# ctu-mrs/mrs_multirotor_simulator

Hardware: NVIDIA B200
Metric: UAV-steps/s (RK4+control+collisions) at 1M UAVs (higher is better)
Workload: dtype f64

## Files before the change

mrs_multirotor_simulator_b200/csrc/api.cu:

```cuda
#include <dlfcn.h>
#include <nccl.h>

#include <algorithm>
#include <cmath>
#include <cstdarg>
#include <cstdio>
#include <cstring>
#include <functional>
#include <map>
#include <memory>
#include <string>
#include <type_traits>
#include <utility>
#include <vector>

#include "internal.h"
#include "params.h"

static thread_local char g_err[512] = "";

static int fail(int code, const char* fmt, ...) {
  va_list ap;
  va_start(ap, fmt);
  vsnprintf(g_err, sizeof(g_err), fmt, ap);
  va_end(ap);
  return code;
}

#define CU(call)                                                                                              \
  do {                                                                                                        \
    cudaError_t e_ = (call);                                                                                  \
    if (e_ != cudaSuccess) return fail(MRSB_ERR_CUDA, "%s failed: %s (%s:%d)", #call, cudaGetErrorString(e_), __FILE__, __LINE__); \
  } while (0)

struct NcclApi {
  void* lib = nullptr;
  ncclResult_t (*GetUniqueId)(ncclUniqueId*)                                                         = nullptr;
  ncclResult_t (*CommInitRank)(ncclComm_t*, int, ncclUniqueId, int)                                  = nullptr;
  ncclResult_t (*CommDestroy)(ncclComm_t)                                                            = nullptr;
  ncclResult_t (*AllGather)(const void*, void*, size_t, ncclDataType_t, ncclComm_t, cudaStream_t)    = nullptr;
  ncclResult_t (*Broadcast)(const void*, void*, size_t, ncclDataType_t, int, ncclComm_t, cudaStream_t) = nullptr;
// ... 167 lines not shown
  bool                 equal_shards = true;

  bool                 p2p       = false;
  double*              gbuf[2]   = {nullptr, nullptr};
  uint32_t*            d_gbox[2] = {nullptr, nullptr};
  int64_t              pass_no   = 0;
  bool                 wrote_since_pass = false;
  std::vector<int32_t> pending_geom[2];
  PeerView             pv[2]{};
  PeerView             pv_local{};
  P2PCtl               p2pctl{};
  unsigned long long*  d_flags   = nullptr;
  unsigned long long** d_peer_flags = nullptr;
  std::vector<void*>   ipc_opened;
  Mem<int, true>       h_status;

  cudaStream_t up_stream = nullptr, down_stream = nullptr;
  Mem<double>  d_up[2];
  Mem<double>  d_snap[2];
  cudaEvent_t  ev_up[2] = {nullptr, nullptr}, ev_applied[2] = {nullptr, nullptr}, ev_snap[2] = {nullptr, nullptr}, ev_down[2] = {nullptr, nullptr};
  uint64_t     n_up = 0, n_down = 0;
  Mem<int32_t> d_sub_idx;
  int64_t      n_sub = 0;

  Graph pass[2], tick[2];
  bool  graph_failed = false;

  bool     lists_on            = false;
  int      steps_since_pass    = 0;
  bool     positions_touched   = true;
  int      rebuild_own         = 0;
  int64_t  list_passes         = 0;
  int64_t  rebuilds_counted    = 0;
  Mem<uint32_t, true> h_one;
  Mem<unsigned long long, true> h_until;

  struct NbWorkspace {
    Mem<double>             pos, vel;
    Mem<uint32_t>           bucket, rank, count, begin;
    Mem<double4>            rec;
    Mem<unsigned long long> scan;
  } nb;

  struct Snapshot {
    Mem<unsigned char> mem;
    bool    filled       = false;
    int32_t uniform_mode = MRSB_INPUT_UNKNOWN;
    bool    any_moment   = false;
  };
  std::map<int32_t, Snapshot> snapshots;
  int32_t                     next_snapshot = 1;

  int64_t n_steps = 0, n_passes = 0, n_launches = 0;
  int     step_info[4] = {0, 0, 0, 0};
};

static std::string set_key(const ParamSet& s) {
  return std::string(reinterpret_cast<const char*>(&s), sizeof(ParamSet));
}

static int intern_set(mrsb_sim* h, const ParamSet& s) {
  const std::string key = set_key(s);
  auto              it  = h->set_index.find(key);
  if (it != h->set_index.end()) return it->second;
  const int id = int(h->sets.size());
  h->sets.push_back(s);
// ... 23 lines not shown
  s.cp.rate_kp = cp.rate_kp, s.cp.rate_kd = cp.rate_kd, s.cp.rate_ki = cp.rate_ki;
  s.cp.att_kp = cp.att_kp, s.cp.att_kd = cp.att_kd, s.cp.att_ki = cp.att_ki, s.cp.att_max_rate_roll_pitch = cp.att_max_rate_roll_pitch,
  s.cp.att_max_rate_yaw = cp.att_max_rate_yaw;
  s.cp.vel_kp = cp.vel_kp, s.cp.vel_kd = cp.vel_kd, s.cp.vel_ki = cp.vel_ki, s.cp.vel_max_acceleration = cp.vel_max_acceleration;
  s.cp.pos_kp = cp.pos_kp, s.cp.pos_kd = cp.pos_kd, s.cp.pos_ki = cp.pos_ki, s.cp.pos_max_velocity = cp.pos_max_velocity;
  return s;
}

static int collect_param_sets(mrsb_sim* h) {
  const int n_sets = int(h->sets.size());
  if (n_sets <= 32) return MRSB_OK;
  std::vector<int> refs(size_t(n_sets), 0);
  for (int32_t id : h->pset_host) refs[size_t(id)]++;
  int live = 0;
  for (int r : refs) live += r > 0;
  if (2 * live > n_sets) return MRSB_OK;
  std::vector<int>      remap(size_t(n_sets), -1);
  std::vector<ParamSet> kept;
  kept.reserve(size_t(live));
  h->set_index.clear();
  for (int k = 0; k < n_sets; k++) {
    if (!refs[size_t(k)]) continue;
    remap[size_t(k)] = int(kept.size());
    h->set_index[set_key(h->sets[size_t(k)])] = int(kept.size());
    kept.push_back(h->sets[size_t(k)]);
  }
  h->sets.swap(kept);
  for (int32_t& id : h->pset_host) id = remap[size_t(id)];
  CU(cudaMemcpyAsync(h->d_pset, h->pset_host.data(), sizeof(int32_t) * h->pset_host.size(), cudaMemcpyHostToDevice, h->stream));
  CU(cudaStreamSynchronize(h->stream));
  return MRSB_OK;
}

static int flush_params(mrsb_sim* h) {
  if (!h->params_dirty) return MRSB_OK;
  int rc = collect_param_sets(h);
  if (rc) return rc;
  const int    n_sets = int(h->sets.size());
  const size_t cap    = size_t(std::max(16, 2 * n_sets));
  rc                  = h->d_params.grow(size_t(n_sets), cap, h->stream);
  if (rc) return rc;
  h->ds.params = h->d_params.get();
  rc           = h->d_takeoff0.grow(size_t(n_sets), cap, h->stream);
  if (rc) return rc;
  std::vector<DevParams> host(n_sets);
  std::vector<uint8_t>   takeoff0(size_t(n_sets), 0);
  for (int k = 0; k < n_sets; k++) {
    mrsb_derive(h->sets[k].mp, h->sets[k].cp, &host[k]);
    takeoff0[size_t(k)] = h->sets[k].mp.takeoff_patch_enabled != 0;
  }
  CU(cudaMemcpyAsync(h->d_params.get(), host.data(), sizeof(DevParams) * n_sets, cudaMemcpyHostToDevice, h->stream));
  CU(cudaMemcpyAsync(h->d_takeoff0.get(), takeoff0.data(), size_t(n_sets), cudaMemcpyHostToDevice, h->stream));
  CU(cudaStreamSynchronize(h->stream));
  h->filt_dt = -1.0;
  for (Bucket& b : h->buckets) {
    int nm = -1, ps = -2;
    for (int64_t k = 0; k < b.count; k++) {
      const int64_t e  = h->inv_host.empty() ? b.slot0 + k : h->inv_host[size_t(b.slot0 + k)];
      const int     id = h->pset_host[size_t(h->ds.shard_begin + e)];
      const int     m  = h->sets[size_t(id)].mp.n_motors;
      if (nm == -1) nm = m;
      if (nm != m) nm = 0;
      if (ps == -2) ps = id;
      if (ps != id) ps = -1;
      if (nm == 0 && ps == -1) break;
    }
    b.nm   = nm > 0 ? nm : 0;
    b.pset = ps >= 0 ? ps : -1;
    if (b.pset >= 0) b.params = host[size_t(b.pset)];
  }
  h->params_dirty = false;
  return MRSB_OK;
}

static int ensure_filt(mrsb_sim* h, double dt) {
  if (h->filt_dt == dt) return MRSB_OK;
  h->n_launches += launch_prep_params(h->d_params.get(), int(h->sets.size()), dt, h->stream);
  for (Bucket& b : h->buckets)
    if (b.pset >= 0) CU(cudaMemcpyAsync(&b.params.filt, &h->d_params.get()[b.pset].filt, sizeof(double), cudaMemcpyDeviceToHost, h->stream));
  CU(cudaStreamSynchronize(h->stream));
  h->filt_dt = dt;
  return MRSB_OK;
}

static int ensure_stage(mrsb_sim* h, size_t bytes) {
  return h->d_stage.grow(bytes, std::max<size_t>(bytes, 1 << 16), h->stream);
}

static int stage_idx(mrsb_sim* h, int64_t n, const int32_t* idx, const int32_t** out) {
  *out = nullptr;
  if (n < 0 || n > h->ds.n && !idx) return fail(MRSB_ERR_INVALID, "n=%lld outside 0..%lld", (long long)n, (long long)h->ds.n);
  if (!idx || n == 0) return MRSB_OK;
  for (int64_t k = 0; k < n; k++)
    if (idx[k] < 0 || idx[k] >= h->ds.n) return fail(MRSB_ERR_INVALID, "idx[%lld]=%d outside 0..%lld", (long long)k, idx[k], (long long)h->ds.n - 1);
  int rc = h->d_idx.grow(size_t(n), std::max<size_t>(size_t(n), 1024), h->stream);
  if (rc) return rc;
  CU(cudaMemcpyAsync(h->d_idx.get(), idx, sizeof(int32_t) * n, cudaMemcpyHostToDevice, h->stream));
  *out = h->d_idx.get();
  return MRSB_OK;
}

struct HostRows {
  const double* rows;
  int           width;
};
// ... 132 lines not shown
      ParamSet s = h->sets[old];
      edit(s, k);
      id        = intern_set(h, canonical(s.mp, s.cp));
      memo[key] = id;
      const mrsb_model_params &a = h->sets[size_t(old)].mp, &b = h->sets[size_t(id)].mp;
      if (a.arm_length != b.arm_length || a.prop_radius != b.prop_radius || a.mass != b.mass) geometry = true;
    }
    ids[size_t(k)]                                 = id;
    h->pset_host[size_t(h->ds.shard_begin + i)] = id;
  }
  if (geometry && h->ds.n_global > h->ds.n && !h->p2p) {
    for (int64_t k = n - 1; k >= 0; k--) h->pset_host[size_t(h->ds.shard_begin + (idx ? idx[k] : k))] = olds[size_t(k)];
    return fail(MRSB_ERR_STATE, "arm length / propeller radius / mass of a sharded handle can only change while its peers read them from this "
                                "GPU (exchange mode 2, mrsb_comm_init_nccl with peer access)");
  }
  h->params_dirty = true;
  rc              = ensure_stage(h, sizeof(int32_t) * size_t(n));
  if (rc) return rc;
  CU(cudaMemcpyAsync(h->d_stage.get(), ids.data(), sizeof(int32_t) * size_t(n), cudaMemcpyHostToDevice, h->stream));
  h->n_launches += launch_set_pset(h->d_pset, n, d_idx, h->ds.shard_begin, reinterpret_cast<const int32_t*>(h->d_stage.get()), h->stream);
  CU(cudaStreamSynchronize(h->stream));
  if (geometry) {
    rc = flush_params(h);
    if (rc) return rc;
    rc = stage_idx(h, n, idx, &d_idx);
    if (rc) return rc;
    rc = geometry_changed(h, n, idx, d_idx);
    if (rc) return rc;
    CU(cudaStreamSynchronize(h->stream));
  }
  return MRSB_OK;
}

static void set_collision_geometry(mrsb_sim* h, bool lists) {
  DevGrid& g  = h->grid;
  h->lists_on = lists;
  double cell = lists ? 6.0 : 4.0;
  if (const char* e = getenv("MRSB_COLLISION_CELL")) cell = std::max(3.5, atof(e));
  g.inv_cell = 1.0 / cell;
  g.reach    = 0.5 * cell;
  const double r_list = g.reach * (1.0 - 1e-6);
  g.list_r2  = r_list * r_list;
  g.skin     = (r_list - 1.7320508075688775) * (1.0 - 1e-6);
  h->ds.disp_max       = lists ? &g.ctl->disp_max_bits : nullptr;
  h->positions_touched = true;
}

static void make_local_view(mrsb_sim* h) {
  PeerView& v = h->pv_local;
  v           = PeerView{};
  v.n_ranks   = 1;
  v.rank      = 0;
  v.begin[0]  = 0;
  v.begin[1]  = h->ds.n_global;
  v.pos[0]    = h->ds.gpos;
  v.geom[0]   = h->d_geom[0];
}

static int setup_p2p(mrsb_sim* h) {
  const int    G     = h->n_ranks;
  const size_t ng    = size_t(h->ds.n_global);
  h->gbuf[0]         = h->ds.gpos;
  int rc             = dalloc(h, &h->gbuf[1], 3 * ng);
  if (rc) return rc;
  CU(cudaMemcpy(h->gbuf[1], h->gbuf[0], sizeof(double) * 3 * ng, cudaMemcpyDeviceToDevice));
  rc = dalloc(h, &h->d_geom[1], 4 * ng);
  if (rc) return rc;
  CU(cudaMemcpy(h->d_geom[1], h->d_geom[0], sizeof(double) * 4 * ng, cudaMemcpyDeviceToDevice));
  for (int k = 0; k < 2; k++) {
    rc = dalloc(h, &h->d_gbox[k], 6 * size_t(h->ds.ld / 32 + 1));
    if (rc) return rc;
  }
  rc = dalloc(h, &h->d_flags, 3 * size_t(G));
  if (rc) return rc;
  rc = h->h_status.alloc(1);
  if (rc) return rc;
  *h->h_status.get() = 0;
  struct Handles {
// ... 49 lines not shown
      h->pv[k].box[r] = static_cast<const uint32_t*>(p);
      rc              = open(all[size_t(r)].geom[k], &p);
      if (rc) return rc;
      h->pv[k].geom[r] = static_cast<const double*>(p);
    }
    rc = open(all[size_t(r)].flags, &p);
    if (rc) return rc;
    pflags[size_t(r)] = static_cast<unsigned long long*>(p);
  }
  rc = dalloc(h, &h->d_peer_flags, size_t(G));
  if (rc) return rc;
  CU(cudaMemcpy(h->d_peer_flags, pflags.data(), sizeof(unsigned long long*) * G, cudaMemcpyHostToDevice));
  Mem<unsigned long long> d_tmp;
  rc = d_tmp.alloc(size_t(G));
  if (rc) return rc;
  NC(g_nccl.AllGather(d_tmp.get() + h->rank, d_tmp.get(), sizeof(unsigned long long), ncclChar, h->comm, h->stream));
  CU(cudaStreamSynchronize(h->stream));
  h->p2pctl.peer_flags = h->d_peer_flags;
  h->p2pctl.flags      = h->d_flags;
  h->p2pctl.n_ranks    = G;
  h->p2pctl.rank       = h->rank;
  h->p2pctl.status     = h->h_status.get();
  {
    const char* e    = getenv("MRSB_P2P_TIMEOUT_MS");
    h->p2pctl.budget = (e ? atoll(e) : 20000LL) * 2000000LL;
  }
  h->p2p     = true;
  h->pass_no = 0;
  h->ds.gpos = h->gbuf[1];
  h->ds.gbox = h->d_gbox[1];
  h->ds.geom = h->d_geom[1];
  h->n_launches += launch_publish_positions(h->ds, h->stream);
  h->wrote_since_pass = true;
  set_collision_geometry(h, h->grid.nl_count != nullptr);
  CU(cudaStreamSynchronize(h->stream));
  return MRSB_OK;
}

extern "C" {

const char* mrsb_last_error(void) {
  return g_err;
}
int mrsb_version(void) {
  return MRSB_VERSION_MAJOR * 1000 + MRSB_VERSION_MINOR;
}

int mrsb_destroy(mrsb_handle h) {
  if (!h) return MRSB_OK;
  cudaSetDevice(h->device);
  const cudaStream_t streams[3] = {h->stream, h->up_stream, h->down_stream};
  for (cudaStream_t s : streams)
    if (s) cudaStreamSynchronize(s);
  for (int k = 0; k < 2; k++) h->pass[k] = Graph(), h->tick[k] = Graph();
  for (void* p : h->ipc_opened) cudaIpcCloseMemHandle(p);
  if (h->comm && g_nccl.CommDestroy) g_nccl.CommDestroy(h->comm);
  for (int k = 0; k < 2; k++)
    for (cudaEvent_t e : {h->ev_up[k], h->ev_applied[k], h->ev_snap[k], h->ev_down[k]})
      if (e) cudaEventDestroy(e);
  delete h;
  for (cudaStream_t s : streams)
    if (s) cudaStreamDestroy(s);
  return MRSB_OK;
}

int mrsb_bucket_layout(int64_t n, int32_t n_types, const int32_t* type_of_local_uav, int32_t* slot_of_uav, int64_t* n_slots, int64_t* bucket_first_slot,
                       int64_t* bucket_count) {
// ... 165 lines not shown
    g.scan_tiles = scan_tiles_for(int64_t(g.n_buckets) + 3);
    g.halo_cap   = std::max<int64_t>(s.n_global - s.n, 1);
    rc = dalloc(h, &g.bucket, ng);
    if (!rc) rc = dalloc(h, &g.rank, ng);
    if (!rc) rc = dalloc(h, &g.count, size_t(g.n_buckets) + 4);
    if (!rc) rc = dalloc(h, &g.begin, size_t(g.n_buckets) + 4);
    if (!rc) rc = dalloc(h, &g.aabb, 6);
    if (!rc) rc = dalloc(h, &g.rec, 2 * ng);
    if (!rc) rc = h->pairs.grow(2 * size_t(g.pair_cap), 2 * size_t(g.pair_cap), h->stream);
    if (!rc) rc = dalloc(h, &g.counters, 4);
    if (!rc) rc = dalloc(h, &g.scan_state, size_t(g.scan_tiles) + size_t(scan_tiles_for(s.n)) + 2);
    if (!rc && s.n_global > s.n) rc = dalloc(h, &g.halo_rec, size_t(g.halo_cap));
    if (!rc && s.n_global > s.n) rc = dalloc(h, &g.halo_bucket, size_t(g.halo_cap));
    if (!rc && s.n_global > s.n) rc = dalloc(h, &g.halo_rank, size_t(g.halo_cap));
    if (!rc) rc = dalloc(h, &g.halo_n, 2);
    if (!rc && s.n_global > s.n) rc = dalloc(h, &g.halo_work, size_t(g.halo_cap / 32 + MRSB_MAX_RANKS + 1));
    if (!rc && getenv("MRSB_TIMELINE")) rc = dalloc(h, &g.tl, size_t(MRSB_TL_TICKS) * 8);
    if (!rc) rc = dalloc(h, &g.ctl, 1);
    if (!rc) rc = h->h_one.alloc(2);
    if (!rc) rc = h->h_until.alloc(1);
    if (rc) return rc;
    g.pairs       = h->pairs.get();
    g.halo_work_n = g.halo_n + 1;
    h->h_one.get()[0] = 1u;
    h->h_one.get()[1] = 0xFFFFFFFFu;
    if (s.n > 0 && !getenv("MRSB_NO_NEIGHBOUR_LISTS")) {
      g.nl_ld = s.ld;
      rc      = dalloc(h, &g.nl_count, size_t(g.nl_ld));
      if (!rc) rc = dalloc(h, &g.nl_items, size_t(MRSB_NL_CAP) * size_t(g.nl_ld));
      if (!rc) rc = dalloc(h, &g.nl_active, size_t(g.nl_ld));
      if (!rc) rc = dalloc(h, &g.act_items, size_t(MRSB_NL_CAP) * size_t(g.nl_ld));
      if (rc) return rc;
    }
    set_collision_geometry(h, g.nl_count != nullptr && s.n_global == s.n);
  }
  make_local_view(h);
  h->shard_begin_of = {s.shard_begin};
  h->shard_count_of = {s.n};
  CU(cudaStreamSynchronize(h->stream));
  *out = guard.release();
  return MRSB_OK;
}

int mrsb_sync(mrsb_handle h) {
  GUARD(h);
  CU(cudaStreamSynchronize(h->stream));
  if (h->up_stream) CU(cudaStreamSynchronize(h->up_stream));
  if (h->down_stream) CU(cudaStreamSynchronize(h->down_stream));
  return MRSB_OK;
}

static int ensure_pipeline(mrsb_sim* h) {
  if (h->d_snap[1].get()) return MRSB_OK;
  for (cudaStream_t* s : {&h->up_stream, &h->down_stream})
    if (!*s) CU(cudaStreamCreateWithFlags(s, cudaStreamNonBlocking));
  const size_t snap = 3 * size_t(std::max<int64_t>(h->ds.n, 1));
  for (int k = 0; k < 2; k++) {
    for (cudaEvent_t* e : {&h->ev_up[k], &h->ev_applied[k], &h->ev_snap[k], &h->ev_down[k]})
      if (!*e) CU(cudaEventCreateWithFlags(e, cudaEventDisableTiming));
    int rc = h->d_snap[k].grow(snap, snap, h->down_stream);
    if (rc) return rc;
  }
  return MRSB_OK;
}

int mrsb_set_input_async(mrsb_handle h, int32_t mode, const double* payload, int32_t stride) {
  GUARD(h);
// ... 1240 lines not shown
```

mrs_multirotor_simulator_b200/csrc/collide.cu:

```cuda
#include <algorithm>

#include "internal.h"

namespace {

#define DEV __device__ __forceinline__

#define NL_LIVE 0x80000000u
#define NL_CROWDED 0x40000000u

DEV unsigned long long now_ns() {
  unsigned long long t;
  asm volatile("mov.u64 %0, %globaltimer;" : "=l"(t));
  return t;
}
DEV void stamp(const DevGrid& g, int slot, unsigned long long value) {
  if (g.tl) g.tl[((g.ctl->n_passes - 1ull) % MRSB_TL_TICKS) * 8 + slot] = value;
}

DEV int cell_of(double v, double inv_cell) {
  return __double2int_rd(__dmul_rn(v, inv_cell));
}

DEV uint32_t row_hash(int cy, int cz) {
  uint32_t h = uint32_t(cy) * 0x9E3779B1u ^ (uint32_t(cz) * 0x85EBCA77u + 0x165667B1u);
  h ^= h >> 15;
  h *= 0x2C1B3C6Du;
  h ^= h >> 12;
  return h;
}

DEV unsigned long long enc(double v) {
  const unsigned long long b = (unsigned long long)__double_as_longlong(v);
  return (b >> 63) ? ~b : (b | 0x8000000000000000ull);
}
DEV double dec(unsigned long long e) {
  const unsigned long long b = (e >> 63) ? (e & 0x7fffffffffffffffull) : ~e;
  return __longlong_as_double((long long)b);
}
DEV float fdec(uint32_t e) {
  return __uint_as_float((e >> 31) ? (e & 0x7fffffffu) : ~e);
}
// ... 196 lines not shown
    double*       lp = s.gpos + 3 * gj;
    lp[0] = x, lp[1] = y, lp[2] = z;
    double2* lg = reinterpret_cast<double2*>(s.geom + 4 * gj);
    lg[0] = a, lg[1] = b;
  }
}

#define SCAN_PER_THREAD 16
#define SCAN_TILE (256 * SCAN_PER_THREAD)
#define SCAN_FLAG_A (1ull << 32)
#define SCAN_FLAG_P (2ull << 32)
template <bool HASWORK>
__global__ void __launch_bounds__(256) scan_kernel(const uint32_t* __restrict__ in, uint32_t* __restrict__ out, int64_t n, unsigned long long* state) {
  __shared__ uint32_t s_tile, s_warp[8], s_prefix;
  const uint32_t      full = 0xffffffffu;
  const int           lane = threadIdx.x & 31, wid = threadIdx.x >> 5;
  if (threadIdx.x == 0) s_tile = uint32_t(atomicAdd(&state[0], 1ull));
  __syncthreads();
  const int64_t tile = s_tile;
  const int64_t base = tile * SCAN_TILE + int64_t(threadIdx.x) * SCAN_PER_THREAD;
  uint32_t      v[SCAN_PER_THREAD];
  if (base + SCAN_PER_THREAD <= n) {
#pragma unroll
    for (int q = 0; q < SCAN_PER_THREAD / 4; q++) {
      const uint4 a = reinterpret_cast<const uint4*>(in + base)[q];
      v[4 * q] = a.x, v[4 * q + 1] = a.y, v[4 * q + 2] = a.z, v[4 * q + 3] = a.w;
    }
  } else {
#pragma unroll
    for (int k = 0; k < SCAN_PER_THREAD; k++) v[k] = base + k < n ? in[base + k] : 0u;
  }
  if (HASWORK) {
#pragma unroll
    for (int k = 0; k < SCAN_PER_THREAD; k++) v[k] = (v[k] & 0x7FFFFFFFu) != 0u ? 1u : 0u;
  }
  uint32_t mine = 0;
#pragma unroll
  for (int k = 0; k < SCAN_PER_THREAD; k++) mine += v[k];
  uint32_t incl = mine;
#pragma unroll
  for (int o = 1; o < 32; o <<= 1) {
    const uint32_t t = __shfl_up_sync(full, incl, o);
    if (lane >= o) incl += t;
  }
  if (lane == 31) s_warp[wid] = incl;
  __syncthreads();
  uint32_t warp_off = 0, total = 0;
#pragma unroll
  for (int w = 0; w < 8; w++) {
    if (w < wid) warp_off += s_warp[w];
    total += s_warp[w];
  }
  if (wid == 0) {
    volatile unsigned long long* st = state + 1;
    uint32_t                     prefix = 0;
    if (tile == 0) {
      if (lane == 0) st[0] = SCAN_FLAG_P | total;
    } else {
      if (lane == 0) st[tile] = SCAN_FLAG_A | total;
      int64_t look = tile - 1;
      while (true) {
        const int64_t      t = look - lane;
        unsigned long long w = t >= 0 ? st[t] : SCAN_FLAG_P;
        while (__any_sync(full, (w >> 32) == 0ull)) {
          if ((w >> 32) == 0ull) w = st[t];
        }
        const uint32_t pm    = __ballot_sync(full, (w >> 32) == 2ull);
// ... 176 lines not shown
  PairAcc acc;
  if (n_ball > 0) {
    const Geom Gi      = load_geom(s, gi);
    auto       process = [&](const double4& r) { process_pair(s, g, crash_mode, rebounce, gi, q.x, q.y, q.z, Gi, __double_as_longlong(r.w), r.x, r.y, r.z, acc); };
    if (n_ball <= 2) {
      for (int c = 0; c < n_ball; c++) {
        process(g.rec[h0]);
        h0 = h1;
      }
    } else {
      int64_t last = -1;
      for (int c = 0; c < n_ball; c++) {
        int64_t  best = INT64_MAX;
        uint32_t bt   = 0;
        for (int k = 0; k < 4; k++) {
          for (uint32_t t = st.lo[k]; t < st.hi[k]; t++) {
            const double4 r  = g.rec[t];
            const int64_t gj = __double_as_longlong(r.w);
            if (gj <= last || gj >= best || !in_ball(r, k)) continue;
            best = gj;
            bt   = t;
          }
        }
        if (best == INT64_MAX) break;
        process(g.rec[bt]);
        last = best;
      }
    }
  }
  store_result(s, li, acc);
  if (g.nl_count) g.nl_count[li] = (g.nl_count[li] & ~NL_LIVE) | (nonzero(acc) ? NL_LIVE : 0u);
}


__global__ void __launch_bounds__(128) build_lists_kernel(DevState s, DevGrid g) {
  if (blockIdx.x == 0 && threadIdx.x == 0) stamp(g, 7, now_ns());
  const uint32_t full  = 0xffffffffu;
  const int      lane  = threadIdx.x & 31;
  const int      k     = threadIdx.x & 3;
  const int64_t  n_rec = int64_t(g.begin[g.n_buckets]);
  const uint32_t quad  = 0xFu << (lane & ~3);
  const uint32_t below = quad & ((1u << lane) - 1u);
  const uint32_t mask  = g.n_buckets - 1;
  const bool     write_all = g.ctl->n_passes <= g.ctl->write_all_until;
  for (int64_t p0 = int64_t(blockIdx.x) * 32; p0 < n_rec; p0 += int64_t(gridDim.x) * 32) {
    const int64_t p   = p0 + (threadIdx.x >> 2);
    const bool    has = p < n_rec;
    double4       q   = make_double4(0.0, 0.0, 0.0, 0.0);
    if (has) q = g.rec[p];
    const int64_t gi   = __double_as_longlong(q.w);
    const int64_t li   = gi - s.shard_begin;
    const bool    mine = has && li >= 0 && li < s.n;
    const int cx0 = cell_of(q.x - g.reach, g.inv_cell), cy0 = cell_of(q.y - g.reach, g.inv_cell), cz0 = cell_of(q.z - g.reach, g.inv_cell);
    uint32_t  lo = 0, len = 0;
    if (mine) {
      const uint32_t b0 = (row_hash(cy0 + (k & 1), cz0 + (k >> 1)) + uint32_t(cx0)) & mask;
      lo                = g.begin[b0];
      len               = g.begin[b0 + 2] - lo;
    }
    const int      qb  = lane & ~3;
    const uint32_t lo0 = __shfl_sync(full, lo, qb), lo1 = __shfl_sync(full, lo, qb + 1), lo2 = __shfl_sync(full, lo, qb + 2), lo3 = __shfl_sync(full, lo, qb + 3);
    const uint32_t c1  = __shfl_sync(full, len, qb);
    const uint32_t c2  = c1 + __shfl_sync(full, len, qb + 1);
    const uint32_t c3  = c2 + __shfl_sync(full, len, qb + 2);
    const uint32_t tot = c3 + __shfl_sync(full, len, qb + 3);
    auto where = [&](uint32_t c, int& row) -> uint32_t {
      row = int(c >= c1) + int(c >= c2) + int(c >= c3);
      return row == 0 ? lo0 + c : (row == 1 ? lo1 + (c - c1) : (row == 2 ? lo2 + (c - c2) : lo3 + (c - c3)));
    };
    uint32_t cnt = 0;
    for (uint32_t c = uint32_t(k); __any_sync(full, c < tot); c += 8) {
      double4 r[2];
      int     row[2] = {0, 0};
#pragma unroll
      for (int u = 0; u < 2; u++)
        if (c + 4 * u < tot) r[u] = g.rec[where(c + 4 * u, row[u])];
#pragma unroll
      for (int u = 0; u < 2; u++) {
        bool    take = false;
        int32_t gj   = 0;
        if (c + 4 * u < tot) {
          gj = int32_t(__double_as_longlong(r[u].w));
          if (int64_t(gj) != gi && nf_dist2(q.x, q.y, q.z, r[u].x, r[u].y, r[u].z) < g.list_r2 && cell_of(r[u].y, g.inv_cell) == cy0 + (row[u] & 1) &&
              cell_of(r[u].z, g.inv_cell) == cz0 + (row[u] >> 1))
            take = true;
        }
        const uint32_t bal = __ballot_sync(full, take) & quad;
        if (take) {
          const uint32_t slot = cnt + __popc(bal & below);
          if (slot < MRSB_NL_CAP) g.nl_items[int64_t(slot) * g.nl_ld + li] = gj;
        }
        cnt += __popc(bal);
      }
    }
    __syncwarp();
    const bool lead = mine && k == 0;
    if (lead) {
      uint32_t live = g.nl_count[li] & NL_LIVE;
      if (cnt == 0u && (live || write_all)) {
        const int64_t sl            = slot_of(s, li);
        s.fext[tix(F3_ROWS, 0, sl)] = 0.0;
        s.fext[tix(F3_ROWS, 1, sl)] = 0.0;
        s.fext[tix(F3_ROWS, 2, sl)] = 0.0;
        live                        = 0u;
      }
      if (cnt > MRSB_NL_CAP) {
        g.nl_items[li] = int32_t(uint32_t(p));
        g.nl_count[li] = NL_CROWDED | live;
        atomicAdd(&g.ctl->n_crowded, 1u);
      } else {
        g.nl_count[li] = cnt | live;
      }
    }
  }
}

__global__ void __launch_bounds__(256) compact_kernel(DevGrid g, const uint32_t* __restrict__ slot, int64_t n) {
  const int64_t li = int64_t(blockIdx.x) * blockDim.x + threadIdx.x;
  if (li >= n) return;
  const uint32_t word = g.nl_count[li];
  const bool     work = (word & 0x7FFFFFFFu) != 0u;
  if (work) {
    const uint32_t k   = slot[li];
    g.nl_active[k]     = make_uint2(uint32_t(li), word);
    const uint32_t cnt = (word & NL_CROWDED) ? 1u : (word & ~(NL_LIVE | NL_CROWDED));
    for (uint32_t c = 0; c < cnt; c++) g.act_items[int64_t(c) * g.nl_ld + k] = g.nl_items[int64_t(c) * g.nl_ld + li];
  }
  if (li == n - 1) g.ctl->n_active = slot[li] + (work ? 1u : 0u);
}

DEV void check_crowded(const DevState& s, const DevGrid& g, int crash_mode, double rebounce, int64_t gi, uint32_t rec_index, PairAcc& acc) {
  const double4 qb = g.rec[rec_index];
  const Stencil st = stencil_of(g, qb.x, qb.y, qb.z);
  const double* qp = s.gpos + 3 * gi;
  const double  qx = qp[0], qy = qp[1], qz = qp[2];
  auto in_ball = [&](const double4& r, int k) {
    const int64_t gj = __double_as_longlong(r.w);
    if (gj == gi) return false;
    if (cell_of(r.y, g.inv_cell) != st.rcy[k] || cell_of(r.z, g.inv_cell) != st.rcz[k]) return false;
    double rx, ry, rz;
    load_pos(s, gj, rx, ry, rz);
    return nf_dist2(qx, qy, qz, rx, ry, rz) < 3.0;
  };
  const Geom Gi      = load_geom(s, gi);
  auto       process = [&](int64_t gj) {
    double rx, ry, rz;
    load_pos(s, gj, rx, ry, rz);
    process_pair(s, g, crash_mode, rebounce, gi, qx, qy, qz, Gi, gj, rx, ry, rz, acc);
  };
  int     n_ball = 0;
  int64_t h0 = 0, h1 = 0;
  for (int k = 0; k < 4; k++)
    for (uint32_t t = st.lo[k]; t < st.hi[k]; t++) {
      const double4 r = g.rec[t];
      if (!in_ball(r, k)) continue;
      if (n_ball == 0) h0 = __double_as_longlong(r.w);
      if (n_ball == 1) h1 = __double_as_longlong(r.w);
      n_ball++;
    }
  if (n_ball <= 2) {
    if (n_ball >= 1) process(h0);
    if (n_ball == 2) process(h1);
    return;
  }
  int64_t last = -1;
  for (int c = 0; c < n_ball; c++) {
    int64_t best = INT64_MAX;
    for (int k = 0; k < 4; k++)
      for (uint32_t t = st.lo[k]; t < st.hi[k]; t++) {
        const double4 r  = g.rec[t];
        const int64_t gj = __double_as_longlong(r.w);
        if (gj <= last || gj >= best || !in_ball(r, k)) continue;
        best = gj;
      }
    if (best == INT64_MAX) break;
    process(best);
    last = best;
  }
}

DEV void check_one(const DevState& s, const DevGrid& g, int crash_mode, double rebounce, uint32_t k, int64_t li, uint32_t word, const int32_t* first4) {
  const uint32_t cnt  = word & ~(NL_LIVE | NL_CROWDED);
  const bool     live = (word & NL_LIVE) || g.ctl->n_passes <= g.ctl->write_all_until;
  PairAcc acc;
  if (word & NL_CROWDED) {
    check_crowded(s, g, crash_mode, rebounce, li + s.shard_begin, uint32_t(first4[0]), acc);
  } else if (cnt) {
    const int64_t gi = li + s.shard_begin;
    const double* qp = s.gpos + 3 * gi;
    const double  qx = qp[0], qy = qp[1], qz = qp[2];
    uint32_t      hits = 0;
    for (uint32_t base = 0; base < cnt; base += 4) {
      int32_t gj[4];
      double  r[4][3];
#pragma unroll
      for (int u = 0; u < 4; u++) gj[u] = base + u < cnt ? (base == 0 ? first4[u] : g.act_items[int64_t(base + u) * g.nl_ld + k]) : -1;
#pragma unroll
      for (int u = 0; u < 4; u++) load_pos(s, int64_t(max(gj[u], 0)), r[u][0], r[u][1], r[u][2]);
#pragma unroll
      for (int u = 0; u < 4; u++)
        if (gj[u] >= 0 && nf_dist2(qx, qy, qz, r[u][0], r[u][1], r[u][2]) < 3.0) hits |= 1u << (base + u);
    }
    if (hits) {
      const Geom Gi      = load_geom(s, gi);
      auto       process = [&](uint32_t c) {
        const int64_t gj = g.act_items[int64_t(c) * g.nl_ld + k];
        double        rx, ry, rz;
        load_pos(s, gj, rx, ry, rz);
        process_pair(s, g, crash_mode, rebounce, gi, qx, qy, qz, Gi, gj, rx, ry, rz, acc);
      };
      if (__popc(hits) <= 2) {
        while (hits) {
          process(uint32_t(__ffs(int(hits)) - 1));
          hits &= hits - 1;
        }
      } else {
        int64_t last = -1;
        while (hits) {
          int64_t  best = INT64_MAX;
          uint32_t bc   = 0;
          for (uint32_t m = hits; m; m &= m - 1) {
            const uint32_t c  = uint32_t(__ffs(int(m)) - 1);
            const int64_t  gj = g.act_items[int64_t(c) * g.nl_ld + k];
            if (gj > last && gj < best) best = gj, bc = c;
          }
          if (best == INT64_MAX) break;
          process(bc);
          last = best;
          hits &= ~(1u << bc);
        }
      }
    }
  }
  const bool nz = nonzero(acc);
  if (live || nz) store_result(s, li, acc);
  else if (acc.crashed_me) s.flags[slot_of(s, li)] |= FLAG_CRASHED;
  if (nz != bool(word & NL_LIVE)) {
    const uint32_t nw = (word & ~NL_LIVE) | (nz ? NL_LIVE : 0u);
    g.nl_count[li]    = nw;
    g.nl_active[k].y  = nw;
  }
}

#ifndef MRSB_CHECK_THREADS
#define MRSB_CHECK_THREADS 256
#define MRSB_CHECK_MINB 4
#endif
__global__ void __launch_bounds__(MRSB_CHECK_THREADS, MRSB_CHECK_MINB) check_kernel(DevState s, DevGrid g, int crash_mode, double rebounce, int skip_if_rebuild) {
  if (skip_if_rebuild && g.ctl->rebuild) return;
  if (blockIdx.x == 0 && threadIdx.x == 0) stamp(g, 4, now_ns());
  const uint32_t n_active = g.ctl->n_active;
  for (uint32_t k = blockIdx.x * blockDim.x + threadIdx.x; k < n_active; k += gridDim.x * blockDim.x) {
    const uint2 e = g.nl_active[k];
    int32_t     first4[4];
#pragma unroll
    for (int u = 0; u < 4; u++) first4[u] = g.act_items[int64_t(u) * g.nl_ld + k];
    check_one(s, g, crash_mode, rebounce, k, int64_t(e.x), e.y, first4);
  }
}

__global__ void __launch_bounds__(32) decide_kernel(NlCtl* __restrict__ c, unsigned long long* __restrict__ pair_counter, double skin, int always,
                                                    cudaGraphConditionalHandle handle, int has_handle, P2PCtl p, unsigned long long* tl) {
  const uint32_t full = 0xffffffffu;
  const int      lane = threadIdx.x;
  unsigned long long* row = tl ? tl + (c->n_passes % MRSB_TL_TICKS) * 8 : nullptr;
  if (row && lane == 0) row[0] = now_ns();
  uint32_t                 bits  = c->disp_max_bits;
  const double             D_old = c->D_total;
  const uint32_t           force = c->force, valid = c->valid;
  const unsigned long long n_rebuilds = c->n_rebuilds, n_passes = c->n_passes;
  if (p.n_ranks > 1) {
    const unsigned long long epoch = c->epoch + 1ull;
    const int                slot  = int(epoch & 1ull);
    const bool               peer  = lane < p.n_ranks && lane != p.rank;
    volatile unsigned long long* theirs = peer ? p.peer_flags[lane] : nullptr;
    if (peer) theirs[p.n_ranks + 2 * p.rank + slot] = (unsigned long long)(always ? 0xFFFFFFFFu : bits);
    __threadfence_system();
    if (peer) theirs[p.rank] = epoch;
    if (row && lane == 0) row[1] = now_ns();
    uint32_t got = 0u;
    if (peer) {
      volatile const unsigned long long* mine = p.flags;
      const long long                    t0   = clock64();
      bool                               ok   = true;
      while (mine[lane] < epoch) {
        if (clock64() - t0 > p.budget) {
          *p.status = 1;
          ok        = false;
          break;
        }
// ... 224 lines not shown
```

mrs_multirotor_simulator_b200/csrc/internal.h:

```cpp
#pragma once
#include <cuda_runtime.h>
#include <stdint.h>

#include "../../include/mrsb.h"

#define MRSB_NM MRSB_MAX_MOTORS
#define MRSB_TILE 128

static __host__ __device__ __forceinline__ int64_t tix(int rows, int row, int64_t i) {
  return ((i >> 7) * rows + row) * MRSB_TILE + (i & (MRSB_TILE - 1));
}
#define ST_ROWS 18
#define VPREV_ROWS 3
#define F3_ROWS 3

#define FLAG_CRASHED 1u
#define FLAG_TAKEOFF 2u
#define FLAG_VPREV 4u
#define FLAG_HAD_INPUT 256u
#define FLAG_FF_VEL_HDG_RATE 16u
#define FLAG_FF_VEL_HDG 32u
#define FLAG_FF_ACC_HDG_RATE 64u
#define FLAG_FF_ACC_HDG 128u

// ... 58 lines not shown
#define STEP_OPT_IMU 1u
#define STEP_OPT_GPOS 2u
#define STEP_OPT_NEED_INPUT 4u

#define MRSB_MAX_RANKS 16
struct PeerView {
  int32_t         n_ranks, rank;
  int64_t         begin[MRSB_MAX_RANKS + 1];
  const double*   pos[MRSB_MAX_RANKS];
  const uint32_t* box[MRSB_MAX_RANKS];
  const double*   geom[MRSB_MAX_RANKS];
};

struct P2PCtl {
  unsigned long long* const* peer_flags;
  unsigned long long*        flags;
  int32_t                    n_ranks, rank;
  int*                       status;
  long long                  budget;
};

#define MRSB_NL_CAP 8
#define MRSB_TL_TICKS 4096
struct NlCtl {
  uint32_t disp_max_bits;
  uint32_t force;
  uint32_t valid;
  uint32_t n_active;
  uint32_t n_crowded;
  uint32_t rebuild;
  double   D_total;
  unsigned long long n_rebuilds, n_passes, epoch ;
  unsigned long long write_all_until;
};

struct DevGrid {
  uint32_t  n_buckets;
  uint32_t  bits;
  double    inv_cell;
  double    reach;
  double    list_r2;
  double    skin;
  uint32_t* nl_count;
  int32_t*  nl_items;
  int64_t   nl_ld;
  uint2*    nl_active;
  int32_t*  act_items;
  NlCtl*    ctl;
  uint32_t* bucket;
  uint32_t* rank;
  uint32_t* count;
  uint32_t* begin;
  double4*  rec;
  unsigned long long* aabb;
  unsigned long long* scan_state;
  int32_t   scan_tiles;
  double4*  halo_rec;
  uint32_t* halo_bucket, *halo_rank;
  uint32_t* halo_n;
  uint32_t* halo_work;
  uint32_t* halo_work_n;
  int64_t   halo_cap;
  unsigned long long* tl;
  int32_t*  pairs;
  int64_t   pair_cap;
  unsigned long long* counters;
// ... 44 lines not shown
```

Before: 6.356 billion.

## Store per-UAV clearance in neighbour lists and skip far-apart entries in check

While building neighbour lists, the kernel records a quantised minimum neighbour distance in spare bits of each count word. The check pass uses it to skip non-live, non-crowded entries whose clearance still exceeds the contact cutoff plus accumulated displacement. Entries that still need a visit are compacted in shared memory so warps stay busy on real work. The cost is extra shared memory, block syncs, and a cutoff computed on the host from arm and prop sizes, with a correctness risk if the bound is wrong.

```diff
diff --git a/mrs_multirotor_simulator_b200/csrc/api.cu b/mrs_multirotor_simulator_b200/csrc/api.cu
--- a/mrs_multirotor_simulator_b200/csrc/api.cu
+++ b/mrs_multirotor_simulator_b200/csrc/api.cu
@@ -7,6 +7,7 @@
 #include <cstdio>
 #include <cstring>
 #include <functional>
+#include <limits>
 #include <map>
 #include <memory>
 #include <string>
@@ -240,6 +241,7 @@
   int      rebuild_own         = 0;
   int64_t  list_passes         = 0;
   int64_t  rebuilds_counted    = 0;
+  bool     contact_cut_off     = false;
   Mem<uint32_t, true> h_one;
   Mem<unsigned long long, true> h_until;
 
@@ -329,6 +331,21 @@
   return MRSB_OK;
 }
 
+static int update_contact_cut(mrsb_sim* h) {
+  if (!h->grid.ctl) return MRSB_OK;
+  double c = 3.0, reach = 0.0;
+  for (const ParamSet& set : h->sets) {
+    const double a = set.mp.arm_length, p = set.mp.prop_radius;
+    if (!(a >= 0.0 && p >= 0.0 && a + p < 1e300)) reach = 1e300;
+    reach = std::max(reach, a + p);
+  }
+  if (h->ds.n_global == h->ds.n) c = std::min(c, 2.0 * reach * (1.0 + 1e-6));
+  if (h->contact_cut_off) c = std::numeric_limits<double>::infinity();
+  CU(cudaMemcpyAsync(&h->grid.ctl->c_cut, &c, sizeof(double), cudaMemcpyHostToDevice, h->stream));
+  CU(cudaStreamSynchronize(h->stream));
+  return MRSB_OK;
+}
+
 static int flush_params(mrsb_sim* h) {
   if (!h->params_dirty) return MRSB_OK;
   int rc = collect_param_sets(h);
@@ -367,7 +384,7 @@
     if (b.pset >= 0) b.params = host[size_t(b.pset)];
   }
   h->params_dirty = false;
-  return MRSB_OK;
+  return update_contact_cut(h);
 }
 
 static int ensure_filt(mrsb_sim* h, double dt) {
@@ -566,7 +583,7 @@
   return MRSB_OK;
 }
 
-static void set_collision_geometry(mrsb_sim* h, bool lists) {
+static int set_collision_geometry(mrsb_sim* h, bool lists) {
   DevGrid& g  = h->grid;
   h->lists_on = lists;
   double cell = lists ? 6.0 : 4.0;
@@ -578,6 +595,7 @@
   g.skin     = (r_list - 1.7320508075688775) * (1.0 - 1e-6);
   h->ds.disp_max       = lists ? &g.ctl->disp_max_bits : nullptr;
   h->positions_touched = true;
+  return update_contact_cut(h);
 }
 
 static void make_local_view(mrsb_sim* h) {
@@ -693,7 +711,8 @@
   h->ds.geom = h->d_geom[1];
   h->n_launches += launch_publish_positions(h->ds, h->stream);
   h->wrote_since_pass = true;
-  set_collision_geometry(h, h->grid.nl_count != nullptr);
+  rc = set_collision_geometry(h, h->grid.nl_count != nullptr);
+  if (rc) return rc;
   CU(cudaStreamSynchronize(h->stream));
   return MRSB_OK;
 }
@@ -925,7 +944,9 @@
       if (!rc) rc = dalloc(h, &g.act_items, size_t(MRSB_NL_CAP) * size_t(g.nl_ld));
       if (rc) return rc;
     }
-    set_collision_geometry(h, g.nl_count != nullptr && s.n_global == s.n);
+    h->contact_cut_off = getenv("MRSB_NO_CONTACT_CUT") != nullptr;
+    rc                 = set_collision_geometry(h, g.nl_count != nullptr && s.n_global == s.n);
+    if (rc) return rc;
   }
   make_local_view(h);
   h->shard_begin_of = {s.shard_begin};
diff --git a/mrs_multirotor_simulator_b200/csrc/collide.cu b/mrs_multirotor_simulator_b200/csrc/collide.cu
--- a/mrs_multirotor_simulator_b200/csrc/collide.cu
+++ b/mrs_multirotor_simulator_b200/csrc/collide.cu
@@ -8,6 +8,10 @@
 
 #define NL_LIVE 0x80000000u
 #define NL_CROWDED 0x40000000u
+#define NL_COUNT 0x0000000Fu
+#define NL_CLR_SHIFT 4
+#define NL_CLR_MAX 0x03FFFFFFu
+#define NL_CLR_UNIT (1.0 / 1048576.0)
 
 DEV unsigned long long now_ns() {
   unsigned long long t;
@@ -270,7 +274,7 @@
   }
   if (HASWORK) {
 #pragma unroll
-    for (int k = 0; k < SCAN_PER_THREAD; k++) v[k] = (v[k] & 0x7FFFFFFFu) != 0u ? 1u : 0u;
+    for (int k = 0; k < SCAN_PER_THREAD; k++) v[k] = (v[k] & (NL_COUNT | NL_CROWDED)) != 0u ? 1u : 0u;
   }
   uint32_t mine = 0;
 #pragma unroll
@@ -513,6 +517,14 @@
   if (g.nl_count) g.nl_count[li] = (g.nl_count[li] & ~NL_LIVE) | (nonzero(acc) ? NL_LIVE : 0u);
 }
 
+
+DEV uint32_t clearance_code(double d2) {
+  const double u = __dmul_rd(__dmul_rd(__dsqrt_rd(d2), 1.0 - 1e-6), 1.0 / NL_CLR_UNIT);
+  return u < double(NL_CLR_MAX) ? uint32_t(u) : NL_CLR_MAX;
+}
+DEV double clearance_of(uint32_t word) {
+  return double((word >> NL_CLR_SHIFT) & NL_CLR_MAX) * NL_CLR_UNIT;
+}
 
 __global__ void __launch_bounds__(128) build_lists_kernel(DevState s, DevGrid g) {
   if (blockIdx.x == 0 && threadIdx.x == 0) stamp(g, 7, now_ns());
@@ -549,7 +561,8 @@
       row = int(c >= c1) + int(c >= c2) + int(c >= c3);
       return row == 0 ? lo0 + c : (row == 1 ? lo1 + (c - c1) : (row == 2 ? lo2 + (c - c2) : lo3 + (c - c3)));
     };
-    uint32_t cnt = 0;
+    uint32_t cnt   = 0;
+    double   d2min = g.list_r2;
     for (uint32_t c = uint32_t(k); __any_sync(full, c < tot); c += 8) {
       double4 r[2];
       int     row[2] = {0, 0};
@@ -561,10 +574,13 @@
         bool    take = false;
         int32_t gj   = 0;
         if (c + 4 * u < tot) {
-          gj = int32_t(__double_as_longlong(r[u].w));
-          if (int64_t(gj) != gi && nf_dist2(q.x, q.y, q.z, r[u].x, r[u].y, r[u].z) < g.list_r2 && cell_of(r[u].y, g.inv_cell) == cy0 + (row[u] & 1) &&
-              cell_of(r[u].z, g.inv_cell) == cz0 + (row[u] >> 1))
-            take = true;
+          gj              = int32_t(__double_as_longlong(r[u].w));
+          const double d2 = nf_dist2(q.x, q.y, q.z, r[u].x, r[u].y, r[u].z);
+          if (int64_t(gj) != gi && d2 < g.list_r2 && cell_of(r[u].y, g.inv_cell) == cy0 + (row[u] & 1) &&
+              cell_of(r[u].z, g.inv_cell) == cz0 + (row[u] >> 1)) {
+            take  = true;
+            d2min = fmin(d2min, d2);
+          }
         }
         const uint32_t bal = __ballot_sync(full, take) & quad;
         if (take) {
@@ -574,6 +590,8 @@
         cnt += __popc(bal);
       }
     }
+    d2min = fmin(d2min, __shfl_xor_sync(full, d2min, 1));
+    d2min = fmin(d2min, __shfl_xor_sync(full, d2min, 2));
     __syncwarp();
     const bool lead = mine && k == 0;
     if (lead) {
@@ -590,7 +608,7 @@
         g.nl_count[li] = NL_CROWDED | live;
         atomicAdd(&g.ctl->n_crowded, 1u);
       } else {
-        g.nl_count[li] = cnt | live;
+        g.nl_count[li] = cnt | (cnt ? clearance_code(d2min) << NL_CLR_SHIFT : 0u) | live;
       }
     }
   }
@@ -600,11 +618,11 @@
   const int64_t li = int64_t(blockIdx.x) * blockDim.x + threadIdx.x;
   if (li >= n) return;
   const uint32_t word = g.nl_count[li];
-  const bool     work = (word & 0x7FFFFFFFu) != 0u;
+  const bool     work = (word & (NL_COUNT | NL_CROWDED)) != 0u;
   if (work) {
     const uint32_t k   = slot[li];
     g.nl_active[k]     = make_uint2(uint32_t(li), word);
-    const uint32_t cnt = (word & NL_CROWDED) ? 1u : (word & ~(NL_LIVE | NL_CROWDED));
+    const uint32_t cnt = (word & NL_CROWDED) ? 1u : (word & NL_COUNT);
     for (uint32_t c = 0; c < cnt; c++) g.act_items[int64_t(c) * g.nl_ld + k] = g.nl_items[int64_t(c) * g.nl_ld + li];
   }
   if (li == n - 1) g.ctl->n_active = slot[li] + (work ? 1u : 0u);
@@ -661,7 +679,7 @@
 }
 
 DEV void check_one(const DevState& s, const DevGrid& g, int crash_mode, double rebounce, uint32_t k, int64_t li, uint32_t word, const int32_t* first4) {
-  const uint32_t cnt  = word & ~(NL_LIVE | NL_CROWDED);
+  const uint32_t cnt  = word & NL_COUNT;
   const bool     live = (word & NL_LIVE) || g.ctl->n_passes <= g.ctl->write_all_until;
   PairAcc acc;
   if (word & NL_CROWDED) {
@@ -723,20 +741,65 @@
   }
 }
 
+DEV double contact_cut(const NlCtl* c) {
+  if (c->n_passes <= c->write_all_until) return __longlong_as_double(0x7FF0000000000000ll);
+  return __dadd_ru(__dsqrt_ru(c->c_cut), __dmul_ru(2.0, c->D_total));
+}
+DEV bool must_visit(uint32_t word, double cut) {
+  return (word & (NL_LIVE | NL_CROWDED)) || !(clearance_of(word) >= cut);
+}
+
 #ifndef MRSB_CHECK_THREADS
 #define MRSB_CHECK_THREADS 256
 #define MRSB_CHECK_MINB 4
 #endif
+#define MRSB_CHECK_ROUNDS 4
+#define MRSB_CHECK_SLOTS (MRSB_CHECK_ROUNDS * MRSB_CHECK_THREADS)
 __global__ void __launch_bounds__(MRSB_CHECK_THREADS, MRSB_CHECK_MINB) check_kernel(DevState s, DevGrid g, int crash_mode, double rebounce, int skip_if_rebuild) {
+  __shared__ uint32_t s_k[MRSB_CHECK_SLOTS], s_n;
+  __shared__ uint2    s_e[MRSB_CHECK_SLOTS];
+  __shared__ int32_t  s_head[4][MRSB_CHECK_SLOTS];
   if (skip_if_rebuild && g.ctl->rebuild) return;
   if (blockIdx.x == 0 && threadIdx.x == 0) stamp(g, 4, now_ns());
-  const uint32_t n_active = g.ctl->n_active;
-  for (uint32_t k = blockIdx.x * blockDim.x + threadIdx.x; k < n_active; k += gridDim.x * blockDim.x) {
-    const uint2 e = g.nl_active[k];
-    int32_t     first4[4];
-#pragma unroll
-    for (int u = 0; u < 4; u++) first4[u] = g.act_items[int64_t(u) * g.nl_ld + k];
-    check_one(s, g, crash_mode, rebounce, k, int64_t(e.x), e.y, first4);
+  const uint32_t full   = 0xffffffffu;
+  const int      lane   = threadIdx.x & 31;
+  const uint32_t stride = gridDim.x * MRSB_CHECK_THREADS;
+  for (uint32_t c0 = blockIdx.x * MRSB_CHECK_THREADS; c0 < g.ctl->n_active; c0 += MRSB_CHECK_ROUNDS * stride) {
+    const uint32_t n_active = g.ctl->n_active;
+    const double   cut      = contact_cut(g.ctl);
+    if (threadIdx.x == 0) s_n = 0u;
+    __syncthreads();
+    for (int r = 0; r < MRSB_CHECK_ROUNDS && c0 + r * stride < n_active; r++) {
+      const uint32_t k    = c0 + r * stride + threadIdx.x;
+      const bool     have = k < n_active;
+      uint2          e    = make_uint2(0u, 0u);
+      int32_t        head[4];
+      if (have) e = g.nl_active[k];
+#pragma unroll
+      for (int u = 0; u < 4; u++) head[u] = have ? g.act_items[int64_t(u) * g.nl_ld + k] : 0;
+      const bool     visit = have && must_visit(e.y, cut);
+      const uint32_t bal   = __ballot_sync(full, visit);
+      uint32_t       base  = 0u;
+      if (lane == 0 && bal) base = atomicAdd(&s_n, uint32_t(__popc(bal)));
+      base = __shfl_sync(full, base, 0);
+      if (visit) {
+        const uint32_t j = base + __popc(bal & ((1u << lane) - 1u));
+        s_k[j]           = k;
+        s_e[j]           = e;
+#pragma unroll
+        for (int u = 0; u < 4; u++) s_head[u][j] = head[u];
+      }
+    }
+    __syncthreads();
+    const uint32_t n_visit = s_n;
+    for (uint32_t j = threadIdx.x; j < n_visit; j += MRSB_CHECK_THREADS) {
+      const uint2 e = s_e[j];
+      int32_t     first4[4];
+#pragma unroll
+      for (int u = 0; u < 4; u++) first4[u] = s_head[u][j];
+      check_one(s, g, crash_mode, rebounce, s_k[j], int64_t(e.x), e.y, first4);
+    }
+    __syncthreads();
   }
 }
 
diff --git a/mrs_multirotor_simulator_b200/csrc/internal.h b/mrs_multirotor_simulator_b200/csrc/internal.h
--- a/mrs_multirotor_simulator_b200/csrc/internal.h
+++ b/mrs_multirotor_simulator_b200/csrc/internal.h
@@ -114,6 +114,7 @@
   double   D_total;
   unsigned long long n_rebuilds, n_passes, epoch ;
   unsigned long long write_all_until;
+  double   c_cut;
 };
 
 struct DevGrid {
```

Measured after the change: 6.536 billion (median of 6 runs). +2.8%, better.
